# qqueing/DeepSpeaker-pytorch

Hardware: AMD Instinct MI355X
Metric: embeddings/sec (64-fbank x 160-frame utterances) (higher is better)
Workload: dtype f16

## Files before the change

### deepspeaker-pytorch_amd/_native.py

```python
from __future__ import annotations

import ctypes
import os
from ctypes import POINTER, Structure, c_char_p, c_double, c_float, c_int, c_longlong, c_void_p

_HERE = os.path.dirname(os.path.abspath(__file__))
LIB_NAME = "libdeepspeaker_hip.so"

DS_EPI_AFFINE, DS_EPI_RESIDUAL, DS_EPI_CLIP, DS_EPI_STATS, DS_EPI_OUT_F32, DS_EPI_OUT_F16 = 1, 2, 4, 8, 16, 32
DS_EPI_OUT_PLANES16, DS_CONV_IN_PLANES16 = 256, 512
DS_CONV_HINT_SINGLE_BUFFER = 64
DS_CONV_HINT_CHUNK16 = 128
DS_CONV_HINT_NO_PERSIST = 1024
DS_CONV_HINT_NO_WIDE = 2048
DS_CONV_HINT_ONE_QUEUE = 4096
DS_CONV_CK = 8
DS_TAIL_SMALL_MAX_B = 4


class ConvShape(Structure):
    _fields_ = [("B", c_int), ("H", c_int), ("W", c_int), ("Cin", c_int),
                ("Cout", c_int), ("KS", c_int), ("stride", c_int)]


class PackJob(Structure):
    _fields_ = [("w_oihw", c_void_p), ("out", c_void_p), ("out2", c_void_p),
                ("Cout", c_int), ("Cin", c_int), ("KS", c_int), ("mode", c_int)]


class DeepSpeakerHipError(RuntimeError):
    pass


_P = c_void_p
_SIGNATURES = {
    "ds_version": (c_int, []),
    "ds_mfma_rate_probe": (c_int, [c_int, c_int, _P, _P, _P]),
    "ds_mfma_rate_probe_data": (c_int, [_P, c_longlong, _P, c_longlong, c_int, _P, _P, _P]),
# ... 9 lines not shown
    "ds_nchw_to_nhwc_f32": (c_int, [_P, _P, c_int, c_int, c_int, c_int, _P]),
    "ds_nhwc_to_nchw_f32": (c_int, [_P, _P, c_int, c_int, c_int, c_int, _P]),
    "ds_pack_conv_weight_f32": (c_int, [_P, _P, c_int, c_int, c_int, c_int, _P]),
    "ds_pack_conv1_weight_f32": (c_int, [_P, _P, c_int, _P]),
    "ds_pack_fc_weight_f32": (c_int, [_P, _P, c_int, c_int, c_int, _P]),
    "ds_pack_fc_weight_dgrad_f32": (c_int, [_P, _P, c_int, c_int, c_int, _P]),
    "ds_bn_fold_f32": (c_int, [_P, _P, _P, _P, c_float, _P, _P, c_int, _P]),
    "ds_bn_stats_finalize_f32": (c_int, [_P, c_int, c_longlong, _P, _P, c_float, c_float, _P, _P, _P, _P,
                                         _P, _P, c_int, _P]),
    "ds_bn_apply_f32": (c_int, [_P, _P, _P, _P, _P, c_longlong, c_int, c_int, _P]),
    "ds_conv_out_dims": (c_int, [POINTER(ConvShape), POINTER(c_int), POINTER(c_int)]),
    "ds_conv_stats_rows": (c_int, [POINTER(ConvShape)]),
    "ds_conv_plan_describe": (c_int, [POINTER(ConvShape), POINTER(c_int)]),
    "ds_conv5x5s2_c1_stats_rows": (c_int, [c_int, c_int]),
    "ds_conv5x5s2_c1_fwd_f32": (c_int, [_P, _P, _P, _P, _P, _P, c_int, c_int, c_int, c_int, c_int, _P]),
    "ds_conv5x5s2_c1_fwd_bf16": (c_int, [_P, _P, _P, _P, _P, _P, c_int, c_int, c_int, c_int, c_int, _P]),
    "ds_conv_fwd_f32": (c_int, [POINTER(ConvShape), _P, _P, _P, _P, _P, _P, _P, c_int, _P]),
    "ds_pack_conv_weight_bf16": (c_int, [_P, _P, _P, c_int, c_int, c_int, _P]),
    "ds_pack_conv_weight_dgrad_bf16": (c_int, [_P, _P, _P, c_int, c_int, c_int, _P]),
    "ds_pack_conv_weight_dgrad_s2_bf16": (c_int, [_P, _P, _P, c_int, c_int, _P]),
    "ds_conv_dgrad_bf16": (c_int, [POINTER(ConvShape), _P, _P, _P, _P, _P]),
    "ds_conv_bf16_stats_rows": (c_int, [POINTER(ConvShape), c_int]),
    "ds_conv_bf16_plan_describe": (c_int, [POINTER(ConvShape), c_int, POINTER(c_int)]),
    "ds_conv_bf16_set_forced_cfg": (None, [c_int]),
    "ds_conv_fwd_bf16": (c_int, [POINTER(ConvShape), _P, _P, _P, _P, _P, _P, _P, _P, c_int, _P]),
    "ds_pack_conv_weight_f16": (c_int, [_P, _P, c_int, c_int, c_int, _P]),
    "ds_pack_conv_weights_f16_batch": (c_int, [POINTER(PackJob), c_int, _P]),
    "ds_pack_conv_weights_bf16_batch": (c_int, [POINTER(PackJob), c_int, _P]),
    "ds_conv_fwd_f16": (c_int, [POINTER(ConvShape), _P, _P, _P, _P, _P, _P, c_int, _P]),
    "ds_conv_f16_splitk_workspace_bytes": (c_longlong, [POINTER(ConvShape)]),
    "ds_conv_fwd_f16_splitk": (c_int, [POINTER(ConvShape), _P, _P, _P, _P, _P, _P, c_int, _P, c_longlong, _P]),
    "ds_conv_block_f16_supported": (c_int, [c_int, c_int, c_int, c_int]),
    "ds_conv_block_f16": (c_int, [_P, _P, _P, _P, _P, _P, _P, _P, c_int, c_int, c_int, c_int, c_int, _P]),
    "ds_conv_block_f16_masked": (c_int, [_P, _P, _P, _P, _P, _P, _P, _P, _P, c_int, c_int, c_int, c_int, c_int, _P]),
    "ds_conv_f16_plan_describe": (c_int, [POINTER(ConvShape), POINTER(c_int)]),
    "ds_conv_f16_plan_describe_hinted": (c_int, [POINTER(ConvShape), c_int, POINTER(c_int)]),
    "ds_conv_f16_set_layout_padding": (None, [c_int]),
    "ds_conv_f16_set_forced_cfg": (None, [c_int]),
    "ds_conv_f16_plan_lds_layout": (c_int, [POINTER(ConvShape), c_int, POINTER(c_int)]),
    "ds_cast_f32_to_f16": (c_int, [_P, _P, c_longlong, _P]),
    "ds_cast_f16_to_f32": (c_int, [_P, _P, c_longlong, _P]),
    "ds_avgpool_time_f32": (c_int, [_P, _P, c_int, c_int, c_int, c_int, _P]),
    "ds_l2norm_scale_f32": (c_int, [_P, _P, c_int, c_int, c_float, c_float, _P]),
    "ds_max_abs_diff_f32": (c_int, [_P, _P, c_longlong, _P, _P]),
    "ds_fc_workspace_floats": (c_longlong, [c_int, c_int, c_int]),
    "ds_fc_l2norm_fwd_f32": (c_int, [_P, _P, _P, _P, _P, _P, c_int, c_int, c_int, c_float, c_float, _P]),
# ... 202 lines not shown
```

### deepspeaker-pytorch_amd/csrc/conv_mfma_bf16.hip

```cpp
#include <ds_device.h>
#include <algorithm>
#include "ds_common.h"

#include "conv_mfma_bf16_kernel.h"
#include "conv_plan.h"

namespace {

__device__ __forceinline__ void pack_conv_weight_bf16_body(const float *w, __bf16 *hi, __bf16 *lo, int Cout, int Cin, int KS,
                                                           int dgrad, int block, int n_blocks) {
    const int T = KS * KS;
    const long long n = (long long)Cout * Cin * T;
    const int N = dgrad ? Cin : Cout;
    for (long long i = (long long)block * 256 + threadIdx.x; i < n; i += (long long)n_blocks * 256) {
        const int kk = (int)(i & 15);
        long long r = i >> 4;
        const int nn = (int)(r % N);
        r /= N;
        const int t = (int)(r % T);
        const int kc = (int)(r / T);
        const int k = kc * 16 + kk;
        const int tt = dgrad ? (T - 1 - t) : t;
        const int kh = tt / KS, kw = tt - kh * KS;
        const int co = dgrad ? k : nn, ci = dgrad ? nn : k;
// ... 29 lines not shown
    double total = 0.0;
    int n = 0;
    for (int m0 = 0; m0 + 32 <= MT; m0 += 32) {
        for (int g = 0; g < 2; ++g) {
            int cnt[16] = {0};
            int worst = 0;
            for (int j = 0; j < 16; ++j) {
                const int m = m0 + 16 * g + j;
                const int seg = m / pix_per_seg, rem = m % pix_per_seg;
                const int r = rem / Wc, c = rem % Wc;
                const int rec = (seg < NI) ? seg * seg_pix + (IS * r) * pitch + c : 0;
                const int slot = (rec * (PSB / 16)) & 15;
                if (++cnt[slot] > worst) worst = cnt[slot];
            }
            total += worst;
            ++n;
        }
    }
    return n ? total / n : 1.0;
}

static int g_forced_cfg_b = -1;

constexpr size_t kLdsSlackB = 16;
static size_t plan_lds_bytes(const TileCfgB &cf, size_t tile_pix, bool x3, int NI) {
    return std::max(tile_pix * PSB * (x3 ? 2 : 1), cf.epi_bytes()) + (size_t)cf.MT() * 4 + (size_t)NI * 8 + (size_t)cf.WM * cf.NTILE() * 8;
}

static int plan_bf16(PlanB &pl, const ds_conv_shape *s, bool x3, int out_stride = 1, int out_h0 = 0, int out_w0 = 0,
                     int out_H = 0, int out_W = 0, int grid_H = 0, int grid_W = 0) {
    int Ho, Wo;
    const int rc = ds_plan_check_shape(s, CKB, false, Ho, Wo, grid_H, grid_W);
    if (rc != DS_OK) return rc;
    const int pad = s->KS / 2;
    const int yH = out_H > 0 ? out_H : Ho, yW = out_W > 0 ? out_W : Wo;
    DS_REQUIRE((long long)s->B * Ho < (1ll << 24), DS_ERR_BAD_SHAPE);
    DS_REQUIRE((long long)s->B * yH * yW * s->Cout < (1ll << 30), DS_ERR_BAD_SHAPE);
    const int IS = s->stride;
    double best = -1.0;
    int bc = -1, brt = 0, bni = 0;
    for (int c = 0; c < kNumCfgB; ++c) {
        const TileCfgB &cf = kCfgB[c];
        if (s->Cout % cf.NTILE()) continue;
        if (cf.x3_only && !x3) continue;
        if (g_forced_cfg_b >= 0 && c != g_forced_cfg_b) continue;
        const long long item_cap = (long long)cf.items_per_thread * cf.NTHR();
        auto fits = [&](int n, int rows_in, int cols_in) {
            return plan_lds_bytes(cf, (size_t)n * rows_in * (cols_in + 4), x3, n) <= cf.lds_cap &&
                   (long long)n * std::min(rows_in, s->H) * s->W * (CKB / 4) <= item_cap;
        };
        ds_plan_segmentations(s->B, Ho, Wo, cf.MT(), IS, s->KS, s->KS, fits, [&](int rt, int ni, long long n_mt) {
            const long long blocks = n_mt * (s->Cout / cf.NTILE());
            double eff = ds_plan_fill_occupancy(s->B, Ho, Wo, n_mt, cf.MT(), blocks, cf.wg_per_cu);
            const long long waves = blocks * (cf.NTHR() / 64);
            if (waves < kPlanSIMDs) eff *= (double)waves / (double)kPlanSIMDs;
            int pref[kNumCfgB] = {0, 2, 7, 8, 5, 6, 1, 4, 3};
#ifdef DS_BF16_PREF_TOP
            pref[DS_BF16_PREF_TOP] = 9;
#endif
            eff += 1e-9 * rt + 1e-6 * pref[c];
            if (eff > best) { best = eff; bc = c; brt = rt; bni = ni; }
        });
    }
    if (bc < 0) return DS_ERR_UNSUPPORTED;
    const TileCfgB &cf = kCfgB[bc];
    ConvKB &k = pl.k;
    k.H = s->H; k.W = s->W; k.Cin = s->Cin;
    k.Hr = Ho; k.Wc = Wo; k.Ho = yH; k.Wo = yW; k.Cout = s->Cout;
    k.OS = out_stride; k.OH0 = out_h0; k.OW0 = out_w0;
    k.IS = IS; k.dh_min = -pad; k.dw_min = -pad;
    pl.cfg = bc;
    ds_plan_fill_geometry(pl, s->B, Ho, Wo, IS, s->KS, s->KS, s->Cout, cf.NTILE(), brt, bni);
    k.half = (k.cols_in + 1) / 2;
    int best_pitch = k.cols_in;
    double best_cost = 1e30;
    for (int pt = k.cols_in; pt <= k.cols_in + 4; ++pt) {
        const double c = frag_read_cost(cf.MT(), bni, brt, Wo, IS, k.rows_in, pt);
        if (c < best_cost - 1e-9) { best_cost = c; best_pitch = pt; }
    }
    k.pitch = best_pitch;
    k.seg_pix = k.rows_in * k.pitch;
    k.y_bytes = (unsigned)((long long)s->B * yH * yW * s->Cout * 4);
    pl.lds_bytes = plan_lds_bytes(cf, (size_t)k.NI * k.seg_pix, x3, k.NI) + kLdsSlackB;
    pl.nit = ds_ceil_div(k.NI * std::min(k.rows_in, s->H) * s->W * (CKB / 4), cf.NTHR());
    k.bn_z = k.bn_mean = k.bn_invstd = k.bn_msc = k.bn_msh = nullptr;
    k.bn_mtiles = 1; k.bn_rows_member = 0; k.bn_row0 = 0;
    return DS_OK;
}

static void set_operands(ConvKB &k, const float *x, const void *w_hi, const void *w_lo, float *y, const float *scale,
                         const float *shift, const float *res, float *stats, int flags) {
    k.x = x; k.w_hi = (const __bf16 *)w_hi; k.w_lo = (const __bf16 *)w_lo; k.y = y;
    k.scale = scale; k.shift = shift; k.res = res; k.stats = stats;
    k.flags = flags;
}

template <int KS, bool X3>
static void launch_b(const PlanB &pl, void *stream) {
    if (KS == 3) { if (X3) ds_bf16_launch_k3x3(pl, stream); else ds_bf16_launch_k3x1(pl, stream); }
    else         { if (X3) ds_bf16_launch_k5x3(pl, stream); else ds_bf16_launch_k5x1(pl, stream); }
}

}

static int pack_job_check(const void *w_oihw, const void *w_hi, int Cout, int Cin, int KS, int dgrad, int bad_ks, long long *n) {
    DS_REQUIRE(w_oihw && w_hi, DS_ERR_NULL);
    DS_REQUIRE((dgrad == 0 || dgrad == 1) && Cout > 0 && Cin > 0, DS_ERR_BAD_SHAPE);
    DS_REQUIRE(KS == 3 || KS == 5, bad_ks);
    DS_REQUIRE((dgrad ? Cout : Cin) % CKB == 0, DS_ERR_BAD_SHAPE);
    *n = (long long)Cout * Cin * KS * KS;
    return DS_OK;
}

static int pack_bf16(const float *w_oihw, void *w_hi, void *w_lo, int Cout, int Cin, int KS, int dgrad, void *stream) {
    long long n;
    const int rc = pack_job_check(w_oihw, w_hi, Cout, Cin, KS, dgrad, DS_ERR_BAD_SHAPE, &n);
    if (rc != DS_OK) return rc;
    long long g = (n + 255) / 256;
    DS_LAUNCH(pack_conv_weight_bf16_kernel, (int)(g > 4096 ? 4096 : g), 256, 0, stream, w_oihw, (__bf16 *)w_hi,
              (__bf16 *)w_lo, Cout, Cin, KS, dgrad);
    return ds_last_launch_error();
// ... 11 lines not shown
        const int rc = pack_job_check(b.w_oihw, b.out, b.Cout, b.Cin, b.KS, b.mode, DS_ERR_UNSUPPORTED, &n);
        if (rc != DS_OK) return rc;
        J.w[j] = b.w_oihw; J.hi[j] = (__bf16 *)b.out; J.lo[j] = (__bf16 *)b.out2;
        J.Cout[j] = b.Cout; J.Cin[j] = b.Cin; J.KS[j] = b.KS; J.dgrad[j] = b.mode;
        const long long g = (n + 255) / 256;
        J.first[j] = blocks;
        blocks += (int)(g > 512 ? 512 : g);
    }
    J.first[n_jobs] = blocks;
    DS_LAUNCH(pack_conv_weight_bf16_batch_kernel, blocks, 256, 0, stream, J);
    return ds_last_launch_error();
}

extern "C" int ds_pack_conv_weight_bf16(const float *w_oihw, void *w_hi, void *w_lo, int Cout, int Cin, int KS,
                                        void *stream) {
    return pack_bf16(w_oihw, w_hi, w_lo, Cout, Cin, KS, 0, stream);
}

extern "C" int ds_pack_conv_weight_dgrad_bf16(const float *w_oihw, void *w_hi, void *w_lo, int Cout, int Cin, int KS,
                                              void *stream) {
    return pack_bf16(w_oihw, w_hi, w_lo, Cout, Cin, KS, 1, stream);
}

extern "C" int ds_conv_bf16_stats_rows(const ds_conv_shape *s, int x3) {
    PlanB pl;
    int rc = plan_bf16(pl, s, x3 != 0);
    return rc == DS_OK ? pl.n_mtiles : rc;
}

extern "C" void ds_conv_bf16_set_forced_cfg(int cfg) { g_forced_cfg_b = (cfg >= 0 && cfg < kNumCfgB) ? cfg : -1; }

extern "C" int ds_conv_bf16_plan_describe(const ds_conv_shape *s, int x3, int *out8) {
    DS_REQUIRE(out8 != nullptr, DS_ERR_NULL);
    PlanB pl;
    int rc = plan_bf16(pl, s, x3 != 0);
    if (rc != DS_OK) return rc;
    const TileCfgB &cf = kCfgB[pl.cfg];
    out8[0] = cf.MT(); out8[1] = cf.NTILE(); out8[2] = pl.k.RT; out8[3] = pl.k.NI;
    out8[4] = pl.grid; out8[5] = (int)pl.lds_bytes; out8[6] = cf.NTHR(); out8[7] = pl.k.pitch;
    return DS_OK;
}

extern "C" int ds_conv_fwd_bf16(const ds_conv_shape *s, const float *x, const void *w_hi, const void *w_lo,
                                const float *scale, const float *shift, const float *residual, float *y,
                                float *stats_partial, int flags, void *stream) {
    DS_REQUIRE(x && w_hi && y, DS_ERR_NULL);
    DS_REQUIRE(!(flags & DS_EPI_AFFINE) || (scale && shift), DS_ERR_NULL);
    DS_REQUIRE(!(flags & DS_EPI_RESIDUAL) || residual, DS_ERR_NULL);
    DS_REQUIRE(!(flags & DS_EPI_STATS) || stats_partial, DS_ERR_NULL);
    DS_REQUIRE(DS_ALIGNED16(x) && DS_ALIGNED16(w_hi) && DS_ALIGNED16(y) && DS_ALIGNED16(w_lo), DS_ERR_ALIGNMENT);
    const bool x3 = w_lo != nullptr;
    PlanB pl;
    int rc = plan_bf16(pl, s, x3);
    if (rc != DS_OK) return rc;
    set_operands(pl.k, x, w_hi, w_lo, y, scale, shift, residual, stats_partial, flags);
    if (s->KS == 3) { if (x3) launch_b<3, true>(pl, stream); else launch_b<3, false>(pl, stream); }
    else            { if (x3) launch_b<5, true>(pl, stream); else launch_b<5, false>(pl, stream); }
    return ds_last_launch_error();
}

__global__ void __launch_bounds__(256) pack_conv_dgrad_s2_bf16_kernel(const float *w, __bf16 *hi, __bf16 *lo, int Cout,
                                                                      int Cin) {
    const long long per_class = (long long)9 * Cout * Cin;
    const long long n = 4 * per_class;
    for (long long i = (long long)blockIdx.x * 256 + threadIdx.x; i < n; i += (long long)gridDim.x * 256) {
        const int cls = (int)(i / per_class);
        long long r = i - cls * per_class;
        const int kk = (int)(r & 15);
        r >>= 4;
        const int ci = (int)(r % Cin);
        r /= Cin;
        const int t = (int)(r % 9);
        const int kc = (int)(r / 9);
        const int co = kc * 16 + kk;
        const int ph = cls >> 1, pw = cls & 1;
        const int dh = t / 3 - 1, dw = t % 3 - 1;
        const int kh = ph + 2 - 2 * dh, kw = pw + 2 - 2 * dw;
        float v = 0.0f;
// ... 156 lines not shown
```

### deepspeaker-pytorch_amd/csrc/conv_mfma_bf16_kernel.h

```cpp
#pragma once
#include <ds_device.h>
#include <type_traits>
#include "ds_common.h"
#include "conv_mfma_f16_parts.h"


constexpr int CKB = 16;
constexpr int PSB = 48;


struct ConvKB {
    const float *x;
    const __bf16 *w_hi, *w_lo;
    float *y;
    const float *scale, *shift, *res;
    float *stats;
    int H, W, Cin;
    int Hr, Wc, Ho, Wo, Cout;
    int IS;
    int dh_min, dw_min;
    int rows_in, cols_in, seg_pix;
    int pitch, half;
    int RT, NI, segs_per_img, n_segs;
    int n_ntiles;
// ... 15 lines not shown
    int MSUB, NSUB, WM, WN;
    int wg_per_cu;
    size_t lds_cap;
    int items_per_thread;
    bool x3_only;
    constexpr int MT() const { return MSUB * WM * 32; }
    constexpr int NTILE() const { return NSUB * WN * 32; }
    constexpr int NTHR() const { return WM * WN * 64; }
    constexpr size_t epi_bytes() const { return (size_t)WM * WN * 32 * (NSUB * 32 + 4) * 4; }
};
constexpr int kNumCfgB = 9;
constexpr TileCfgB kCfgB[kNumCfgB] = {
    {2, 1, 2, 2, 3, 64 * 1024, 16, false},
    {5, 1, 1, 4, 2, 64 * 1024, 16, false},
    {4, 1, 2, 2, 2, 64 * 1024, 16, false},
    {5, 2, 1, 2, 2, 80 * 1024, 32, true},
    {5, 2, 1, 4, 1, 160 * 1024 - 64, 32, true},
    {5, 2, 2, 2, 1, 160 * 1024 - 64, 32, true},
    {5, 2, 2, 1, 2, 80 * 1024, 32, true},
    {4, 2, 1, 2, 2, 80 * 1024, 32, true},
    {4, 2, 1, 4, 1, 160 * 1024 - 64, 32, true},
};

void ds_bf16_launch_k3x3(const PlanB &pl, void *stream);
void ds_bf16_launch_k5x3(const PlanB &pl, void *stream);
void ds_bf16_launch_k3x1(const PlanB &pl, void *stream);
void ds_bf16_launch_k5x1(const PlanB &pl, void *stream);
void ds_bf16_launch_k3x3g(const PlanB &pl, void *stream);

#ifdef DS_BF16_KERNEL_TU
namespace {

template <int KS, int MSUB, int NSUB, int WM, int WN, bool X3, int NIT, bool PREF, bool BNB = false>
__global__ void __launch_bounds__(WM * WN * 64) conv_mfma_bf16_kernel(const ConvKB p) {
    constexpr int NTHR = WM * WN * 64;
    constexpr int MT = MSUB * WM * 32;
    constexpr int NTILE = NSUB * WN * 32;
    constexpr int NT = KS * KS;
    constexpr int RING = (KS == 3) ? (MSUB <= 2 ? 9 : 3) : (KS == 5 ? 5 : 1);
    constexpr bool APREF = (MSUB * NSUB >= 8);
    constexpr bool ILV = X3 && APREF;

    char *lds = (char *)ds_dynamic_lds();
    const int tid = threadIdx.x, lane = tid & 63, wave = tid >> 6;
    const int wm = wave / WN, wn = wave % WN;
    const int l31 = lane & 31, lhi = lane >> 5;
    const int tile_n = blockIdx.x % p.n_ntiles;
    const int tile_m = blockIdx.x / p.n_ntiles;
    const int seg0 = tile_m * p.NI;
    const int pix_per_seg = p.RT * p.Wc;
    const int tile_pix = p.NI * p.seg_pix;
// ... 445 lines not shown
    else if (pl.nit <= 16)
        DS_LAUNCH_BIG_LDS((conv_mfma_bf16_kernel<KS, MSUB, NSUB, WM, WN, true, 16, true, BNB>), pl.grid, NTHR, pl.lds_bytes, stream, pl.k);
    else
        DS_LAUNCH_BIG_LDS((conv_mfma_bf16_kernel<KS, MSUB, NSUB, WM, WN, true, 32, false, BNB>), pl.grid, NTHR, pl.lds_bytes, stream, pl.k);
}

template <int N = 0, class F>
static void ds_bf16_with_cfg(int cfg, F &&f) {
    if constexpr (N < kNumCfgB) {
        if (cfg == N) f(std::integral_constant<int, N>{});
        else ds_bf16_with_cfg<N + 1>(cfg, f);
    }
}

template <int KS, bool X3, bool BNB = false>
static void launch_b(const PlanB &pl, void *stream) {
    ds_bf16_with_cfg(pl.cfg, [&](auto c) {
        constexpr TileCfgB cf = kCfgB[decltype(c)::value];
        if constexpr (!cf.x3_only) launch_nit_b<KS, cf.MSUB, cf.NSUB, cf.WM, cf.WN, X3, BNB>(pl, stream);
        else if constexpr (X3) launch_big_b<KS, cf.MSUB, cf.NSUB, cf.WM, cf.WN, BNB>(pl, stream);
    });
}

}
#endif
```

### deepspeaker-pytorch_amd/engine.py

```python
from __future__ import annotations

import ctypes
import os
from dataclasses import dataclass, field
from typing import Dict, List, Optional, Tuple

import torch

from ._native import (ConvShape, DS_CONV_IN_PLANES16, DS_EPI_AFFINE, DS_EPI_CLIP, DS_EPI_OUT_F16, DS_EPI_OUT_F32,
                      DS_EPI_OUT_PLANES16, DS_EPI_RESIDUAL, DS_EPI_STATS, DS_TAIL_SMALL_MAX_B, NativeLib, PackJob)

PACK_BATCH_MAX = 32

PRECISIONS = ("f32", "bf16x3", "bf16", "f16")

STAGE_CHANNELS = (64, 128, 256, 512)
BN_EPS = 1e-5
BN_MOMENTUM = 0.1
L2_EPS = 1e-10
ALPHA = 10.0


def conv_out(n: int, k: int, stride: int) -> int:
    return (n + 2 * (k // 2) - k) // stride + 1


@dataclass
class BNParams:
    weight: torch.Tensor
    bias: torch.Tensor
    running_mean: torch.Tensor
    running_var: torch.Tensor

# ... 376 lines not shown
        pooled = torch.empty((B, wc * c), dtype=torch.float32, device=a.device)
        self.lib.call("ds_avgpool_time_f32", self._p(a), self._p(pooled), B, hr, wc, c, self._stream(a))
        n_out = pw.fc_bias.numel()
        k = wc * c
        ws_floats = self.lib.raw("ds_fc_workspace_floats")(B, k, n_out)
        if ws_floats <= 0:
            raise RuntimeError(f"ds_fc_workspace_floats({B},{k},{n_out}) failed: {ws_floats}")
        ws = torch.empty(ws_floats, dtype=torch.float32, device=a.device)
        f = torch.empty((B, n_out), dtype=torch.float32, device=a.device)
        e = torch.empty_like(f)
        self.lib.call("ds_fc_l2norm_fwd_f32", self._p(pooled), self._p(pw.fc), self._p(pw.fc_bias.detach()),
                      self._p(ws), self._p(f), self._p(e), B, k, n_out, ALPHA, L2_EPS, self._stream(a))
        if saved is not None:
            saved.pooled, saved.fc_out = pooled, f
        return e

    def _build_eval_plan(self, x, pw: PackedWeights, folded, precision: str, masked: bool = False,
                         low_latency: bool = False, per_layer: bool = False, taps: Optional[dict] = None):
        B, _, T, F = x.shape
        dev = x.device
        lowp = precision != "f32"
        x3 = precision == "bf16x3"
        h16 = precision == "f16"
        x_slot, e_slot, st_slot = ctypes.c_void_p(0), ctypes.c_void_p(0), ctypes.c_void_p(0)
        calls = []
        keep = []
        AC = DS_EPI_AFFINE | DS_EPI_CLIP
        lens_dev = torch.zeros((len(pw.stages), B), dtype=torch.int32, device=dev) if masked else None

        def mask_call(t, stage, hh):
            if masked:
                row_bytes = t.shape[2] * t.shape[3] * t.element_size()
                calls.append((self.lib.raw("ds_mask_rows"), (self._p(t), self._p(lens_dev[stage]), B, hh, row_bytes, st_slot),
                              None, 0.0))

        def buf(*shape, dtype=torch.float32):
            t = torch.empty(shape, dtype=dtype, device=dev)
            keep.append(t)
            return t

        def conv_call(src_p, w_f32, w_bf16, Bc, h, w, cin, cout, ks, stride, sc, sh, res, w_f16=None, last=False,
                      layout_flags=0):
            shp = ConvShape(Bc, h, w, cin, cout, ks, stride)
            keep.append(shp)
            ho, wo = conv_out(h, ks, stride), conv_out(w, ks, stride)
            flags = AC | (DS_EPI_RESIDUAL if res is not None else 0) | layout_flags
            label = f"conv{ks}x{ks}s{stride}_{cin}to{cout}_{ho}x{wo}"
            flops = 2.0 * Bc * ho * wo * cout * cin * ks * ks
            if h16:
                y = buf(Bc, ho, wo, cout, dtype=torch.float32 if last else torch.float16)
                ws_bytes = self.lib.raw("ds_conv_f16_splitk_workspace_bytes")(ctypes.byref(shp)) if low_latency else 0
                if ws_bytes > 0:
                    ws = buf(ws_bytes // 4)
                    args = (ctypes.byref(shp), src_p, self._p(w_f16), self._p(sc), self._p(sh), self._p(res), self._p(y),
                            flags | (DS_EPI_OUT_F32 if last else 0), self._p(ws), ws_bytes, st_slot)
                    calls.append((self.lib.raw("ds_conv_fwd_f16_splitk"), args, label, flops))
                    return y, ho, wo
                args = (ctypes.byref(shp), src_p, self._p(w_f16), self._p(sc), self._p(sh), self._p(res), self._p(y),
                        flags | (DS_EPI_OUT_F32 if last else 0), st_slot)
                calls.append((self.lib.raw("ds_conv_fwd_f16"), args, label, flops))
                return y, ho, wo
            y = buf(Bc, ho, wo, cout)
            if lowp:
                args = (ctypes.byref(shp), src_p, self._p(w_bf16[0]), self._p(w_bf16[1]) if x3 else None,
                        self._p(sc), self._p(sh), self._p(res), self._p(y), None, flags, st_slot)
                calls.append((self.lib.raw("ds_conv_fwd_bf16"), args, label, flops))
            else:
                args = (ctypes.byref(shp), src_p, self._p(w_f32), self._p(sc), self._p(sh), self._p(res), self._p(y),
                        None, flags, st_slot)
                calls.append((self.lib.raw("ds_conv_fwd_f32"), args, label, flops))
            return y, ho, wo

        h, w, cin = T, F, 1
        a = None
        planes = h16 and not low_latency and not per_layer and len(pw.stages) > 1
        for s, sw in enumerate(pw.stages):
            i, c = s + 1, STAGE_CHANNELS[s]
            sc, sh = folded[f"model.bn{i}"]
            if i == 1:
                ho, wo = conv_out(h, 5, 2), conv_out(w, 5, 2)
                a = buf(B, ho, wo, 64, dtype=torch.float16 if h16 else torch.float32)
                calls.append((self.lib.raw("ds_conv5x5s2_c1_fwd_bf16" if precision != "f32" else "ds_conv5x5s2_c1_fwd_f32"),
                              (x_slot, self._p(sw.conv), self._p(sc), self._p(sh), self._p(a), None, B, h, w, 64,
                               AC | (DS_EPI_OUT_F16 if h16 else 0), st_slot), None, 0.0))
                h, w = ho, wo
            else:
                a, h, w = conv_call(self._p(a), sw.conv, sw.conv_bf16, B, h, w, cin, c, 5, 2, sc, sh, None, sw.conv_f16,
                                    layout_flags=DS_CONV_IN_PLANES16 if (planes and i == 2) else 0)
# ... 75 lines not shown
            raise ValueError(f"unknown precision {precision!r}; expected one of {PRECISIONS}")
        if precision == "f16":
            if pw.stages[0].l_conv1_f16 is None:
                raise ValueError("pack_weights(..., with_f16=True) is required for precision 'f16'")
        elif precision != "f32" and pw.stages[0].l_conv1_bf16 is None:
            raise ValueError("pack_weights(..., with_bf16=True) is required for the bf16 precisions")

    def forward_eval_planned(self, x: torch.Tensor, pw: PackedWeights, folded, precision: str = "f32",
                             lengths: Optional[torch.Tensor] = None, low_latency: bool = False) -> torch.Tensor:
        self._check_eval_args(x, pw, precision)
        stream_id = torch.cuda.current_stream(x.device).cuda_stream if x.is_cuda else 0
        key = (tuple(x.shape), precision, id(pw), id(folded), x.device, stream_id, lengths is not None, low_latency)
        plans = self.__dict__.setdefault("_eval_plans", {})
        plan = plans.pop(key, None)
        if plan is not None:
            plans[key] = plan
        if plan is None:
            owner = getattr(pw, "owner", None)
            for k in [k for k, q in plans.items()
                      if k[1] == key[1] and k[4] == key[4] and k[2:4] != key[2:4]
                      and (q.get("owner") is None or q.get("owner") == owner)]:
                del plans[k]
            plan = self._build_eval_plan(x, pw, folded, precision, masked=lengths is not None,
                                         low_latency=low_latency and precision == "f16")
            plan["bytes"] = sum(t.numel() * t.element_size() for t in plan["keep"] if isinstance(t, torch.Tensor))
            plan["owner"] = owner
            while plans and (len(plans) >= self.PLAN_CACHE_ENTRIES
                             or sum(q["bytes"] for q in plans.values()) + plan["bytes"] > self.PLAN_CACHE_BYTES):
                del plans[next(iter(plans))]
            plans[key] = plan
        if lengths is not None:
            ln = lengths.to(torch.int64).cpu()
            if ln.numel() != x.shape[0] or int(ln.min()) < 1 or int(ln.max()) > x.shape[2]:
                raise ValueError("lengths must hold one frame count in [1, T] per utterance of the padded batch")
            per_stage = []
            for _ in range(len(pw.stages)):
                ln = (ln - 1) // 2 + 1
                per_stage.append(ln)
            host = torch.stack(per_stage).to(torch.int32)
            if x.is_cuda:
                host = host.pin_memory()
            plan["lens"].copy_(host, non_blocking=True)
            plan["lens_host"] = host
        prof = self.profile if (self.profile is not None and x.is_cuda) else None
        if prof is not None and self.profile_every > 1:
            turn = self._profile_calls.get(precision, 0)
            self._profile_calls[precision] = turn + 1
# ... 308 lines not shown
```

### deepspeaker-pytorch_amd/mining.py

```python
from __future__ import annotations


import torch

from .model import _require_cuda, get_engine


REFINE_BAND = 1.25e-3
BAND_SAFETY = 2.5
BAND_VIOLATION = 0.5
BAND_WINDOW = 512
PROBE_STRIDE = 37
REFINE_CAP_START = 32
REFINE_CAP_MIN = 4
REFINE_CAP = REFINE_CAP_START


def _pow2ceil(v: int) -> int:
    return 1 << max(0, int(v) - 1).bit_length()


class RefinePolicy:

    HISTORY = 8
    RING = 256

    WARM = 4

    def __init__(self, cap_min: int = REFINE_CAP_MIN, cap_start: int = REFINE_CAP_START,
                 band_floor: float = REFINE_BAND, band_safety: float = BAND_SAFETY):
        self.cap_min, self.cap_start = cap_min, max(cap_min, cap_start)
        self.band_floor, self.band_safety = float(band_floor), float(band_safety)
        self.n_seen = 0
        self.seen = []
        self.errs = []
        self.err_samples = 0
        self.err_max_ever = 0.0
        self.emb_errs = []
# ... 112 lines not shown
        if len(self.entries) >= self.window:
            self.flush()

    def flush(self):
        ents, self.entries = self.entries, []
        if not ents:
            return
        if self.policy.batch is self:
            self.policy.batch = None
        eng, cap = self.eng, self.cap
        dev = self.xr.device
        cur = torch.cuda.current_stream(dev)
        side = _side_stream(dev) if self.side else cur
        for en in ents:
            side.wait_event(en["gathered"])
        with torch.cuda.stream(side):
            if side != cur or any(en["stream"] != side for en in ents):
                self.xr.record_stream(side)
                for en in ents:
                    for v in list(en["t"].values()) + [en["a"], en["p"], en["n"]]:
                        if isinstance(v, torch.Tensor):
                            v.record_stream(side)
            st = eng._stream(self.xr)
            e_ref = eng.forward_eval_planned(self.xr[:len(ents) * 3 * cap], self.pw_ref, self.folded_ref, precision="bf16x3")
            for k, en in enumerate(ents):
                t, a, p, n = en["t"], en["a"], en["p"], en["n"]
                e_k = e_ref[k * 3 * cap:(k + 1) * 3 * cap]
                d_p, d_n = torch.empty_like(t["d_p"]), torch.empty_like(t["d_n"])
                err = torch.empty(5, dtype=torch.float32, device=dev)
                eng.lib.call("ds_refine_distances_fused_f32", eng._p(e_k), eng._p(t["amb_idx"]), eng._p(t["amb_count"]), cap,
                             eng._p(d_p), eng._p(d_n), eng._p(t["d_p"]), eng._p(t["d_n"]), eng._p(a), eng._p(p), eng._p(n),
                             d_p.numel(), a.shape[1], eng._p(err), st)
                rb = self.policy.readback(t["amb_count"], err)
                idx, count = torch.empty_like(t["idx"]), torch.empty_like(t["count"])
                mean_diff, loss = torch.empty_like(t["mean_diff"]), torch.empty_like(t["loss"])
                eng.lib.call("ds_triplet_scan_f32", eng._p(d_p), eng._p(d_n), en["margin"], eng._p(loss), eng._p(idx),
                             eng._p(count), eng._p(mean_diff), d_p.numel(), st)
                en["sel"]._complete(idx, count, d_p, d_n, mean_diff, loss, rb)
            ready = side.record_event()
        for en in ents:
            en["sel"]._ready = ready


class TripletSelection:

    def __init__(self, idx_full, count, d_p, d_n, mean_diff, loss=None, amb_count=None, amb_cap=0, ready=None,
                 readback=None, fallback=None, policy=None, band=0.0):
# ... 176 lines not shown
                               readback=None, fallback=embed_all, policy=policy, band=band)
        sel._window, sel._resolved = w, False
        w.add(t, xs, a, p, n, margin, sel)
        return sel
    if policy.batch is not None:
        policy.batch.flush()
    if side_stream:
        side.wait_stream(main)
    with torch.cuda.stream(side):
        if side_stream:
            for v in list(t.values()) + xs + [a, p, n]:
                if isinstance(v, torch.Tensor):
                    v.record_stream(side)
        if whole:
            rb = policy.readback(t["amb_count"])
            r = embed_all()
            idx, count, d_p, d_n, mean_diff, loss = r["idx"], r["count"], r["d_p"], r["d_n"], r["mean_diff"], r["loss"]
        else:
            rows = xs[0][0].numel()
            xr = torch.empty((3 * cap,) + tuple(xs[0].shape[1:]), dtype=torch.float32, device=a.device)
            st = eng._stream(a)
            eng.lib.call("ds_gather_rows3_f32", eng._p(xs[0]), eng._p(xs[1]), eng._p(xs[2]), eng._p(t["amb_idx"]), eng._p(xr), cap,
                         rows, st)
            e_ref = eng.forward_eval_planned(xr, pw_ref, folded_ref, precision="bf16x3")
            d_p, d_n = torch.empty_like(t["d_p"]), torch.empty_like(t["d_n"])
            err = torch.empty(5, dtype=torch.float32, device=a.device)
            eng.lib.call("ds_refine_distances_fused_f32", eng._p(e_ref), eng._p(t["amb_idx"]), eng._p(t["amb_count"]), cap,
                         eng._p(d_p), eng._p(d_n), eng._p(t["d_p"]), eng._p(t["d_n"]), eng._p(a), eng._p(p), eng._p(n),
                         d_p.numel(), a.shape[1], eng._p(err), st)
            rb = policy.readback(t["amb_count"], err)
            idx, count = torch.empty_like(t["idx"]), torch.empty_like(t["count"])
            mean_diff, loss = torch.empty_like(t["mean_diff"]), torch.empty_like(t["loss"])
            eng.lib.call("ds_triplet_scan_f32", eng._p(d_p), eng._p(d_n), float(margin), eng._p(loss), eng._p(idx),
                         eng._p(count), eng._p(mean_diff), d_p.numel(), st)
        ready = side.record_event()
    return TripletSelection(idx, count, d_p, d_n, mean_diff, loss, t["amb_count"], cap, ready if side_stream else None,
                            readback=rb, fallback=None if whole else embed_all, policy=policy, band=band)


class MinedNegatives:

    def __init__(self, idx, dist, ready):
        self._idx, self._dist, self._ready = idx, dist, ready

    def wait(self):
        if self._ready is not None:
            cur = torch.cuda.current_stream(self._idx.device)
# ... 42 lines not shown
```

### include/deepspeaker_hip.h

```cpp
#ifndef DEEPSPEAKER_HIP_H
#define DEEPSPEAKER_HIP_H

#include <stddef.h>
#include <stdint.h>

#ifdef __cplusplus
extern "C" {
#endif

#define DS_OK               0
#define DS_ERR_BAD_SHAPE   (-1)
#define DS_ERR_ALIGNMENT   (-2)
#define DS_ERR_NULL        (-3)
#define DS_ERR_UNSUPPORTED (-4)
#define DS_ERR_NO_WORKSPACE (-5)

#define DS_EPI_AFFINE   1
#define DS_EPI_RESIDUAL 2
#define DS_EPI_CLIP     4
#define DS_EPI_STATS    8

#define DS_EPI_OUT_F32  16
#define DS_EPI_OUT_F16  32

#define DS_EPI_OUT_PLANES16  256
#define DS_CONV_IN_PLANES16  512
#define DS_CONV_HINT_SINGLE_BUFFER 64
#define DS_CONV_HINT_CHUNK16      128
#define DS_CONV_HINT_NO_WIDE     2048
#define DS_CONV_HINT_ONE_QUEUE   4096
#define DS_CONV_HINT_NO_PERSIST  1024

#define DS_CONV_CK      8

int ds_version(void);
int ds_event_create(void **out_event);
int ds_event_destroy(void *event);
int ds_event_elapsed_ms(void *start, void *stop, float *ms);
int ds_launch_timing_arm(void *start, void *stop);
int ds_launch_timing_end(void);
const char *ds_error_string(int code);

size_t ds_sched_workspace_bytes(void);
int ds_sched_set_workspace(void *zeroed_device_memory, size_t bytes);
long long ds_sched_free_slots(void);
int ds_mfma_rate_probe(int bf16, int iters, float *sink, double *flop_out, void *stream);
int ds_mfma_rate_probe_data(const void *a_f16, long long n_a, const void *b_f16, long long n_b, int iters, float *sink,
                            double *flop_out, void *stream);

// ... 35 lines not shown

int ds_conv_plan_describe(const ds_conv_shape *s, int *out8);
int ds_conv5x5s2_c1_stats_rows(int B, int H);
int ds_conv5x5s2_c1_fwd_f32(const float *x, const float *w_packed, const float *scale,
                            const float *shift, float *y, float *stats_partial, int B, int H,
                            int W, int Cout, int flags, void *stream);
int ds_conv5x5s2_c1_fwd_bf16(const float *x, const float *w_packed, const float *scale,
                             const float *shift, void *y, float *stats_partial, int B, int H,
                             int W, int Cout, int flags, void *stream);
int ds_conv_fwd_f32(const ds_conv_shape *s, const float *x, const float *w_packed,
                    const float *scale, const float *shift, const float *residual, float *y,
                    float *stats_partial, int flags, void *stream);

int ds_pack_conv_weight_bf16(const float *w_oihw, void *w_hi, void *w_lo, int Cout, int Cin, int KS,
                             void *stream);
int ds_pack_conv_weight_dgrad_bf16(const float *w_oihw, void *w_hi, void *w_lo, int Cout, int Cin,
                                   int KS, void *stream);
int ds_pack_conv_weight_dgrad_s2_bf16(const float *w_oihw, void *w_hi, void *w_lo, int Cout, int Cin,
                                      void *stream);
int ds_conv_dgrad_bf16(const ds_conv_shape *s, const float *gy, const void *w_hi, const void *w_lo,
                       float *gx, void *stream);
int ds_conv_bf16_stats_rows(const ds_conv_shape *s, int x3);
int ds_conv_bf16_plan_describe(const ds_conv_shape *s, int x3, int *out8);
void ds_conv_bf16_set_forced_cfg(int cfg);
int ds_conv_fwd_bf16(const ds_conv_shape *s, const float *x, const void *w_hi, const void *w_lo,
                     const float *scale, const float *shift, const float *residual, float *y,
                     float *stats_partial, int flags, void *stream);

int ds_pack_conv_weight_f16(const float *w_oihw, void *w_f16, int Cout, int Cin, int KS, void *stream);
int ds_conv_fwd_f16(const ds_conv_shape *s, const void *x_f16, const void *w_f16, const float *scale,
                    const float *shift, const void *residual_f16, void *y, int flags, void *stream);
long long ds_conv_f16_splitk_workspace_bytes(const ds_conv_shape *s);
int ds_conv_fwd_f16_splitk(const ds_conv_shape *s, const void *x_f16, const void *w_f16, const float *scale,
                           const float *shift, const void *residual_f16, void *y, int flags, void *workspace,
                           long long ws_bytes, void *stream);
int ds_conv_f16_plan_describe(const ds_conv_shape *s, int *out8);
int ds_conv_f16_plan_describe_hinted(const ds_conv_shape *s, int flags, int *out8);
int ds_conv_f16_plan_lds_layout(const ds_conv_shape *s, int flags, int *out4);
void ds_conv_f16_set_layout_padding(int on);
void ds_conv_f16_set_forced_cfg(int cfg);
int ds_conv_block_f16_supported(int B, int H, int W, int C);
int ds_conv_block_f16(const void *x_f16, const void *wa_f16, const void *wb_f16, const float *scale_a,
                      const float *shift_a, const float *scale_b, const float *shift_b, void *y, int B, int H, int W,
                      int C, int flags, void *stream);
int ds_conv_block_f16_masked(const void *x_f16, const void *wa_f16, const void *wb_f16, const float *scale_a,
                             const float *shift_a, const float *scale_b, const float *shift_b, void *y, const int *lens,
// ... 250 lines not shown
```

Before: 396,100.

## Add latency-oriented small-tile bf16x3 conv configs for triplet-mining refinement

```diff
diff --git a/deepspeaker-pytorch_amd/_native.py b/deepspeaker-pytorch_amd/_native.py
--- a/deepspeaker-pytorch_amd/_native.py
+++ b/deepspeaker-pytorch_amd/_native.py
@@ -14,6 +14,7 @@
 DS_CONV_HINT_NO_PERSIST = 1024
 DS_CONV_HINT_NO_WIDE = 2048
 DS_CONV_HINT_ONE_QUEUE = 4096
+DS_CONV_PLAN_LATENCY = 8192
 DS_CONV_CK = 8
 DS_TAIL_SMALL_MAX_B = 4
 
@@ -69,6 +70,7 @@
     "ds_conv_dgrad_bf16": (c_int, [POINTER(ConvShape), _P, _P, _P, _P, _P]),
     "ds_conv_bf16_stats_rows": (c_int, [POINTER(ConvShape), c_int]),
     "ds_conv_bf16_plan_describe": (c_int, [POINTER(ConvShape), c_int, POINTER(c_int)]),
+    "ds_conv_bf16_plan_describe_hinted": (c_int, [POINTER(ConvShape), c_int, c_int, POINTER(c_int)]),
     "ds_conv_bf16_set_forced_cfg": (None, [c_int]),
     "ds_conv_fwd_bf16": (c_int, [POINTER(ConvShape), _P, _P, _P, _P, _P, _P, _P, _P, c_int, _P]),
     "ds_pack_conv_weight_f16": (c_int, [_P, _P, c_int, c_int, c_int, _P]),
diff --git a/deepspeaker-pytorch_amd/csrc/conv_mfma_bf16.hip b/deepspeaker-pytorch_amd/csrc/conv_mfma_bf16.hip
--- a/deepspeaker-pytorch_amd/csrc/conv_mfma_bf16.hip
+++ b/deepspeaker-pytorch_amd/csrc/conv_mfma_bf16.hip
@@ -75,13 +75,16 @@
 
 static int g_forced_cfg_b = -1;
 
+constexpr int kPlanLatRows = 1;
+constexpr int kPlanLatency = 2;
+
 constexpr size_t kLdsSlackB = 16;
 static size_t plan_lds_bytes(const TileCfgB &cf, size_t tile_pix, bool x3, int NI) {
     return std::max(tile_pix * PSB * (x3 ? 2 : 1), cf.epi_bytes()) + (size_t)cf.MT() * 4 + (size_t)NI * 8 + (size_t)cf.WM * cf.NTILE() * 8;
 }
 
 static int plan_bf16(PlanB &pl, const ds_conv_shape *s, bool x3, int out_stride = 1, int out_h0 = 0, int out_w0 = 0,
-                     int out_H = 0, int out_W = 0, int grid_H = 0, int grid_W = 0) {
+                     int out_H = 0, int out_W = 0, int grid_H = 0, int grid_W = 0, int mode = 0) {
     int Ho, Wo;
     const int rc = ds_plan_check_shape(s, CKB, false, Ho, Wo, grid_H, grid_W);
     if (rc != DS_OK) return rc;
@@ -92,11 +95,13 @@
     const int IS = s->stride;
     double best = -1.0;
     int bc = -1, brt = 0, bni = 0;
-    for (int c = 0; c < kNumCfgB; ++c) {
-        const TileCfgB &cf = kCfgB[c];
-        if (s->Cout % cf.NTILE()) continue;
-        if (cf.x3_only && !x3) continue;
-        if (g_forced_cfg_b >= 0 && c != g_forced_cfg_b) continue;
+    long long bwaves = 0, bcost = 0, bblocks = 0;
+    bool latency = false;
+    auto search = [&](int c) {
+        const TileCfgB &cf = ds_bf16_cfg(c);
+        if (s->Cout % cf.NTILE()) return;
+        if (cf.x3_only && !x3) return;
+        if (g_forced_cfg_b >= 0 && c != g_forced_cfg_b) return;
         const long long item_cap = (long long)cf.items_per_thread * cf.NTHR();
         auto fits = [&](int n, int rows_in, int cols_in) {
             return plan_lds_bytes(cf, (size_t)n * rows_in * (cols_in + 4), x3, n) <= cf.lds_cap &&
@@ -107,16 +112,33 @@
             double eff = ds_plan_fill_occupancy(s->B, Ho, Wo, n_mt, cf.MT(), blocks, cf.wg_per_cu);
             const long long waves = blocks * (cf.NTHR() / 64);
             if (waves < kPlanSIMDs) eff *= (double)waves / (double)kPlanSIMDs;
-            int pref[kNumCfgB] = {0, 2, 7, 8, 5, 6, 1, 4, 3};
+            int pref[kNumCfgBAll] = {0, 2, 7, 8, 5, 6, 1, 4, 3, 0, 0};
 #ifdef DS_BF16_PREF_TOP
             pref[DS_BF16_PREF_TOP] = 9;
 #endif
             eff += 1e-9 * rt + 1e-6 * pref[c];
-            if (eff > best) { best = eff; bc = c; brt = rt; bni = ni; }
+            bool better = eff > best;
+            const long long cost = ds_ceil_div_ll(waves, kPlanSIMDs) * ((x3 ? 3 : 1) * cf.MSUB * cf.NSUB);
+            if (latency && bc >= 0) {
+                const TileCfgB &bf = ds_bf16_cfg(bc);
+                const int area = cf.MT() * cf.NTILE(), barea = bf.MT() * bf.NTILE();
+                if (cost != bcost) better = cost < bcost;
+                else if (area != barea) better = area > barea;
+                else if (blocks != bblocks) better = blocks < bblocks;
+            }
+            if (better) { best = eff; bc = c; brt = rt; bni = ni; bwaves = waves; bcost = cost; bblocks = blocks; }
         });
+    };
+    const bool forced_lat = (mode & kPlanLatRows) && g_forced_cfg_b >= kNumCfgB;
+    for (int c = 0; c < (forced_lat ? kNumCfgBAll : kNumCfgB); ++c) search(c);
+    if ((mode & kPlanLatency) && x3 && g_forced_cfg_b < 0 && bc >= 0 && bwaves < kPlanSIMDs) {
+        latency = true;
+        best = -1.0;
+        bc = -1;
+        for (int c = 0; c < kNumCfgBAll; ++c) search(c);
     }
     if (bc < 0) return DS_ERR_UNSUPPORTED;
-    const TileCfgB &cf = kCfgB[bc];
+    const TileCfgB &cf = ds_bf16_cfg(bc);
     ConvKB &k = pl.k;
     k.H = s->H; k.W = s->W; k.Cin = s->Cin;
     k.Hr = Ho; k.Wc = Wo; k.Ho = yH; k.Wo = yW; k.Cout = s->Cout;
@@ -150,6 +172,10 @@
 
 template <int KS, bool X3>
 static void launch_b(const PlanB &pl, void *stream) {
+    if (pl.cfg >= kNumCfgB) {
+        if (KS == 3) ds_bf16_launch_k3x3l(pl, stream); else ds_bf16_launch_k5x3l(pl, stream);
+        return;
+    }
     if (KS == 3) { if (X3) ds_bf16_launch_k3x3(pl, stream); else ds_bf16_launch_k3x1(pl, stream); }
     else         { if (X3) ds_bf16_launch_k5x3(pl, stream); else ds_bf16_launch_k5x1(pl, stream); }
 }
@@ -207,20 +233,26 @@
     return pack_bf16(w_oihw, w_hi, w_lo, Cout, Cin, KS, 1, stream);
 }
 
+static int fwd_plan_mode(int flags) { return kPlanLatRows | ((flags & DS_CONV_PLAN_LATENCY) ? kPlanLatency : 0); }
+
 extern "C" int ds_conv_bf16_stats_rows(const ds_conv_shape *s, int x3) {
     PlanB pl;
-    int rc = plan_bf16(pl, s, x3 != 0);
+    int rc = plan_bf16(pl, s, x3 != 0, 1, 0, 0, 0, 0, 0, 0, fwd_plan_mode(0));
     return rc == DS_OK ? pl.n_mtiles : rc;
 }
 
-extern "C" void ds_conv_bf16_set_forced_cfg(int cfg) { g_forced_cfg_b = (cfg >= 0 && cfg < kNumCfgB) ? cfg : -1; }
+extern "C" void ds_conv_bf16_set_forced_cfg(int cfg) { g_forced_cfg_b = (cfg >= 0 && cfg < kNumCfgBAll) ? cfg : -1; }
 
 extern "C" int ds_conv_bf16_plan_describe(const ds_conv_shape *s, int x3, int *out8) {
+    return ds_conv_bf16_plan_describe_hinted(s, x3, 0, out8);
+}
+
+extern "C" int ds_conv_bf16_plan_describe_hinted(const ds_conv_shape *s, int x3, int flags, int *out8) {
     DS_REQUIRE(out8 != nullptr, DS_ERR_NULL);
     PlanB pl;
-    int rc = plan_bf16(pl, s, x3 != 0);
-    if (rc != DS_OK) return rc;
-    const TileCfgB &cf = kCfgB[pl.cfg];
+    int rc = plan_bf16(pl, s, x3 != 0, 1, 0, 0, 0, 0, 0, 0, fwd_plan_mode(flags));
+    if (rc != DS_OK) return rc;
+    const TileCfgB &cf = ds_bf16_cfg(pl.cfg);
     out8[0] = cf.MT(); out8[1] = cf.NTILE(); out8[2] = pl.k.RT; out8[3] = pl.k.NI;
     out8[4] = pl.grid; out8[5] = (int)pl.lds_bytes; out8[6] = cf.NTHR(); out8[7] = pl.k.pitch;
     return DS_OK;
@@ -233,12 +265,13 @@
     DS_REQUIRE(!(flags & DS_EPI_AFFINE) || (scale && shift), DS_ERR_NULL);
     DS_REQUIRE(!(flags & DS_EPI_RESIDUAL) || residual, DS_ERR_NULL);
     DS_REQUIRE(!(flags & DS_EPI_STATS) || stats_partial, DS_ERR_NULL);
+    DS_REQUIRE(!((flags & DS_CONV_PLAN_LATENCY) && (flags & DS_EPI_STATS)), DS_ERR_UNSUPPORTED);
     DS_REQUIRE(DS_ALIGNED16(x) && DS_ALIGNED16(w_hi) && DS_ALIGNED16(y) && DS_ALIGNED16(w_lo), DS_ERR_ALIGNMENT);
     const bool x3 = w_lo != nullptr;
     PlanB pl;
-    int rc = plan_bf16(pl, s, x3);
-    if (rc != DS_OK) return rc;
-    set_operands(pl.k, x, w_hi, w_lo, y, scale, shift, residual, stats_partial, flags);
+    int rc = plan_bf16(pl, s, x3, 1, 0, 0, 0, 0, 0, 0, fwd_plan_mode(flags));
+    if (rc != DS_OK) return rc;
+    set_operands(pl.k, x, w_hi, w_lo, y, scale, shift, residual, stats_partial, flags & ~DS_CONV_PLAN_LATENCY);
     if (s->KS == 3) { if (x3) launch_b<3, true>(pl, stream); else launch_b<3, false>(pl, stream); }
     else            { if (x3) launch_b<5, true>(pl, stream); else launch_b<5, false>(pl, stream); }
     return ds_last_launch_error();
diff --git a/deepspeaker-pytorch_amd/csrc/conv_mfma_bf16_k3x3l.hip b/deepspeaker-pytorch_amd/csrc/conv_mfma_bf16_k3x3l.hip
--- /dev/null
+++ b/deepspeaker-pytorch_amd/csrc/conv_mfma_bf16_k3x3l.hip
@@ -0,0 +1,4 @@
+#define DS_BF16_KERNEL_TU
+#include "conv_mfma_bf16_kernel.h"
+
+void ds_bf16_launch_k3x3l(const PlanB &pl, void *stream) { launch_lat_b<3>(pl, stream); }
diff --git a/deepspeaker-pytorch_amd/csrc/conv_mfma_bf16_k5x3l.hip b/deepspeaker-pytorch_amd/csrc/conv_mfma_bf16_k5x3l.hip
--- /dev/null
+++ b/deepspeaker-pytorch_amd/csrc/conv_mfma_bf16_k5x3l.hip
@@ -0,0 +1,4 @@
+#define DS_BF16_KERNEL_TU
+#include "conv_mfma_bf16_kernel.h"
+
+void ds_bf16_launch_k5x3l(const PlanB &pl, void *stream) { launch_lat_b<5>(pl, stream); }
diff --git a/deepspeaker-pytorch_amd/csrc/conv_mfma_bf16_kernel.h b/deepspeaker-pytorch_amd/csrc/conv_mfma_bf16_kernel.h
--- a/deepspeaker-pytorch_amd/csrc/conv_mfma_bf16_kernel.h
+++ b/deepspeaker-pytorch_amd/csrc/conv_mfma_bf16_kernel.h
@@ -61,11 +61,21 @@
     {4, 2, 1, 4, 1, 160 * 1024 - 64, 32, true},
 };
 
+constexpr int kNumCfgBLat = 2;
+constexpr TileCfgB kCfgBLat[kNumCfgBLat] = {
+    {1, 1, 2, 2, 2, 64 * 1024, 16, true},
+    {1, 1, 1, 4, 2, 64 * 1024, 16, true},
+};
+constexpr int kNumCfgBAll = kNumCfgB + kNumCfgBLat;
+constexpr const TileCfgB &ds_bf16_cfg(int cfg) { return cfg < kNumCfgB ? kCfgB[cfg] : kCfgBLat[cfg - kNumCfgB]; }
+
 void ds_bf16_launch_k3x3(const PlanB &pl, void *stream);
 void ds_bf16_launch_k5x3(const PlanB &pl, void *stream);
 void ds_bf16_launch_k3x1(const PlanB &pl, void *stream);
 void ds_bf16_launch_k5x1(const PlanB &pl, void *stream);
 void ds_bf16_launch_k3x3g(const PlanB &pl, void *stream);
+void ds_bf16_launch_k3x3l(const PlanB &pl, void *stream);
+void ds_bf16_launch_k5x3l(const PlanB &pl, void *stream);
 
 #ifdef DS_BF16_KERNEL_TU
 namespace {
@@ -557,5 +567,15 @@
     });
 }
 
+template <int KS, int N = 0>
+static void launch_lat_b(const PlanB &pl, void *stream) {
+    if constexpr (N < kNumCfgBLat) {
+        constexpr TileCfgB cf = kCfgBLat[N];
+        static_assert(cf.NTHR() == 256, "launch_nit_b launches 256 threads");
+        if (pl.cfg - kNumCfgB == N) launch_nit_b<KS, cf.MSUB, cf.NSUB, cf.WM, cf.WN, true>(pl, stream);
+        else launch_lat_b<KS, N + 1>(pl, stream);
+    }
+}
+
 }
 #endif
diff --git a/deepspeaker-pytorch_amd/engine.py b/deepspeaker-pytorch_amd/engine.py
--- a/deepspeaker-pytorch_amd/engine.py
+++ b/deepspeaker-pytorch_amd/engine.py
@@ -7,8 +7,8 @@
 
 import torch
 
-from ._native import (ConvShape, DS_CONV_IN_PLANES16, DS_EPI_AFFINE, DS_EPI_CLIP, DS_EPI_OUT_F16, DS_EPI_OUT_F32,
-                      DS_EPI_OUT_PLANES16, DS_EPI_RESIDUAL, DS_EPI_STATS, DS_TAIL_SMALL_MAX_B, NativeLib, PackJob)
+from ._native import (ConvShape, DS_CONV_IN_PLANES16, DS_CONV_PLAN_LATENCY, DS_EPI_AFFINE, DS_EPI_CLIP, DS_EPI_OUT_F16,
+                      DS_EPI_OUT_F32, DS_EPI_OUT_PLANES16, DS_EPI_RESIDUAL, DS_EPI_STATS, DS_TAIL_SMALL_MAX_B, NativeLib, PackJob)
 
 PACK_BATCH_MAX = 32
 
@@ -431,6 +431,8 @@
         lowp = precision != "f32"
         x3 = precision == "bf16x3"
         h16 = precision == "f16"
+        latency_tiles = low_latency and x3
+        low_latency = low_latency and h16
         x_slot, e_slot, st_slot = ctypes.c_void_p(0), ctypes.c_void_p(0), ctypes.c_void_p(0)
         calls = []
         keep = []
@@ -472,7 +474,8 @@
             y = buf(Bc, ho, wo, cout)
             if lowp:
                 args = (ctypes.byref(shp), src_p, self._p(w_bf16[0]), self._p(w_bf16[1]) if x3 else None,
-                        self._p(sc), self._p(sh), self._p(res), self._p(y), None, flags, st_slot)
+                        self._p(sc), self._p(sh), self._p(res), self._p(y), None,
+                        flags | (DS_CONV_PLAN_LATENCY if latency_tiles else 0), st_slot)
                 calls.append((self.lib.raw("ds_conv_fwd_bf16"), args, label, flops))
             else:
                 args = (ctypes.byref(shp), src_p, self._p(w_f32), self._p(sc), self._p(sh), self._p(res), self._p(y),
@@ -594,7 +597,7 @@
                       and (q.get("owner") is None or q.get("owner") == owner)]:
                 del plans[k]
             plan = self._build_eval_plan(x, pw, folded, precision, masked=lengths is not None,
-                                         low_latency=low_latency and precision == "f16")
+                                         low_latency=low_latency)
             plan["bytes"] = sum(t.numel() * t.element_size() for t in plan["keep"] if isinstance(t, torch.Tensor))
             plan["owner"] = owner
             while plans and (len(plans) >= self.PLAN_CACHE_ENTRIES
diff --git a/deepspeaker-pytorch_amd/mining.py b/deepspeaker-pytorch_amd/mining.py
--- a/deepspeaker-pytorch_amd/mining.py
+++ b/deepspeaker-pytorch_amd/mining.py
@@ -14,6 +14,7 @@
 REFINE_CAP_START = 32
 REFINE_CAP_MIN = 4
 REFINE_CAP = REFINE_CAP_START
+REFINE_LOW_LATENCY = True
 
 
 def _pow2ceil(v: int) -> int:
@@ -172,7 +173,8 @@
                         if isinstance(v, torch.Tensor):
                             v.record_stream(side)
             st = eng._stream(self.xr)
-            e_ref = eng.forward_eval_planned(self.xr[:len(ents) * 3 * cap], self.pw_ref, self.folded_ref, precision="bf16x3")
+            e_ref = eng.forward_eval_planned(self.xr[:len(ents) * 3 * cap], self.pw_ref, self.folded_ref, precision="bf16x3",
+                                             low_latency=REFINE_LOW_LATENCY)
             for k, en in enumerate(ents):
                 t, a, p, n = en["t"], en["a"], en["p"], en["n"]
                 e_k = e_ref[k * 3 * cap:(k + 1) * 3 * cap]
@@ -395,7 +397,7 @@
             st = eng._stream(a)
             eng.lib.call("ds_gather_rows3_f32", eng._p(xs[0]), eng._p(xs[1]), eng._p(xs[2]), eng._p(t["amb_idx"]), eng._p(xr), cap,
                          rows, st)
-            e_ref = eng.forward_eval_planned(xr, pw_ref, folded_ref, precision="bf16x3")
+            e_ref = eng.forward_eval_planned(xr, pw_ref, folded_ref, precision="bf16x3", low_latency=REFINE_LOW_LATENCY)
             d_p, d_n = torch.empty_like(t["d_p"]), torch.empty_like(t["d_n"])
             err = torch.empty(5, dtype=torch.float32, device=a.device)
             eng.lib.call("ds_refine_distances_fused_f32", eng._p(e_ref), eng._p(t["amb_idx"]), eng._p(t["amb_count"]), cap,
diff --git a/include/deepspeaker_hip.h b/include/deepspeaker_hip.h
--- a/include/deepspeaker_hip.h
+++ b/include/deepspeaker_hip.h
@@ -25,6 +25,7 @@
 
 #define DS_EPI_OUT_PLANES16  256
 #define DS_CONV_IN_PLANES16  512
+#define DS_CONV_PLAN_LATENCY 8192
 #define DS_CONV_HINT_SINGLE_BUFFER 64
 #define DS_CONV_HINT_CHUNK16      128
 #define DS_CONV_HINT_NO_WIDE     2048
@@ -106,6 +107,7 @@
                        float *gx, void *stream);
 int ds_conv_bf16_stats_rows(const ds_conv_shape *s, int x3);
 int ds_conv_bf16_plan_describe(const ds_conv_shape *s, int x3, int *out8);
+int ds_conv_bf16_plan_describe_hinted(const ds_conv_shape *s, int x3, int flags, int *out8);
 void ds_conv_bf16_set_forced_cfg(int cfg);
 int ds_conv_fwd_bf16(const ds_conv_shape *s, const float *x, const void *w_hi, const void *w_lo,
                      const float *scale, const float *shift, const float *residual, float *y,
```

Measured after the change: 403,300 (median of 6 runs). 1.02x the previous value.
